# TheCacophonyProject/classifier-pipeline

Hardware: AMD Instinct MI355X
Metric: CPTV frames/s end-to-end (track+classify) at 160x120 (higher is better)
Workload: dtype u16/i32 track stage (f32 normalise, f64 gates); f32 crop/tile; f32 CNN (stride-1 3x3 convs of stages 2-4 (+ the stride-2 one): two fp16 planes per operand rounded to nearest (11 + 11 significand bits), power-of-two range scaling, 3 fp16 MFMAs per K step, device-side rerun in the exact split if an ac

## Files before the change

classifier-pipeline_amd/csrc/cpx_cnn_rw.hip:

```cpp
#include <hip/hip_runtime.h>

#include <algorithm>
#include <type_traits>

#include "cpx_conv_layout_core.h"
#include "cpx_kernels.h"

namespace cpx {

namespace {

typedef unsigned u32x4 __attribute__((ext_vector_type(4)));
typedef float f32x4 __attribute__((ext_vector_type(4)));
typedef _Float16 f16x2 __attribute__((ext_vector_type(2)));
typedef _Float16 f16x8 __attribute__((ext_vector_type(8)));

template <typename T>
__device__ __forceinline__ const T* at_off(const T* base, unsigned bytes) {
  return reinterpret_cast<const T*>(reinterpret_cast<const char*>(base) + bytes);
}
template <typename T>
__device__ __forceinline__ T* at_off(T* base, unsigned bytes) {
  return reinterpret_cast<T*>(reinterpret_cast<char*>(base) + bytes);
}
__device__ __forceinline__ unsigned pix_off(int y, int x, int W, int C) {
  return __umul24(__umul24((unsigned)y, (unsigned)W) + (unsigned)x, (unsigned)C);
}
__device__ __forceinline__ float relu_bits(float x) { return __int_as_float(max(__float_as_int(x), 0)); }
__device__ __forceinline__ void split_h(float a, float b, unsigned& hi, unsigned& lo) {
  f16x2 v = {(_Float16)a, (_Float16)b};
  hi = __builtin_bit_cast(unsigned, v);
  asm("v_fma_mixlo_f16 %0, %1, 1.0, -%2 op_sel:[0,0,0] op_sel_hi:[0,0,1]" : "=v"(lo) : "v"(a), "v"(hi));
  asm("v_fma_mixhi_f16 %0, %1, 1.0, -%2 op_sel:[0,0,1] op_sel_hi:[0,0,1]" : "+v"(lo) : "v"(b), "v"(hi));
}
__device__ __forceinline__ f32x4 mfma_h(u32x4 w, u32x4 x, f32x4 c) {
  return __builtin_amdgcn_mfma_f32_16x16x32_f16(__builtin_bit_cast(f16x8, w), __builtin_bit_cast(f16x8, x), c, 0, 0, 0);
}

struct RwTiles {
  unsigned long long m_tx, m_ty;
  int tiles_x, tiles_y, total;
};
template <int I, int N, typename F>
__device__ __forceinline__ void static_for(F&& f) {
  if constexpr (I < N) {
    f(std::integral_constant<int, I>{});
    static_for<I + 1, N>(f);
  }
}
__device__ __forceinline__ int div_magic(int n, unsigned long long m) { return (int)(((unsigned long long)n * m) >> 42); }

constexpr int RW_TW = 16;
constexpr int RW_CT = 256;
constexpr int RW_PPI = RW_CT / 8;
constexpr int RW_WC = 64;

template <int S, int NCH, int ROWS>
struct RwGeo {
  static constexpr int PW = 15 * S + 3, PH = (ROWS - 1) * S + 3, NPX = PH * PW;
  static constexpr int NP = (NPX * 8 + RW_CT - 1) / RW_CT;
  static constexpr int NPXP = (NP * RW_PPI + 3) / 4 * 4 + 2;
  static constexpr int BUF = 2 * 2 * NPXP * 2;
  static constexpr int STEPS = 3 * PH;
  static constexpr int CING = 32 * NCH;
  static constexpr size_t LDS = (size_t)2 * BUF * 16 + (size_t)(2 * CING + 3 * RW_WC) * sizeof(float);
};
constexpr int SC_NPXP = 258;
constexpr int SC_ITEMS = 16 * RW_TW * 8 / RW_CT;
constexpr size_t SC_LDS = (size_t)2 * 2 * SC_NPXP * 2 * 16;

template <int S, int NCH, int ROWS, bool BN, bool RES, bool SC = false>
__global__ __launch_bounds__(RW_CT) __attribute__((amdgpu_waves_per_eu(1, 1))) void conv_rw_kernel(ConvArgs a, const uint4* __restrict__ wimg, RwTiles td) {
  using G = RwGeo<S, NCH, ROWS>;
  constexpr int PW = G::PW, NPX = G::NPX, NP = G::NP, NPXP = G::NPXP, BUF = G::BUF, STEPS = G::STEPS, CING = G::CING, PH = G::PH;
  static_assert(!SC || (S == 1 && NCH == 2 && ROWS == 16 && !RES), "the fp16 shortcut is built into the stride-1 form's two-chunk stream");
  if (*a.ovf != 0) return;
  extern __shared__ __attribute__((aligned(16))) uint4 lds4[];
  uint4* s_buf = lds4;
  float* s_bn = reinterpret_cast<float*>(lds4 + 2 * BUF);
  float* s_par = s_bn + 2 * CING;
  uint4* s_sc = reinterpret_cast<uint4*>(s_par + 3 * RW_WC);
  const int tid = threadIdx.x, lane = tid & 63, wave = tid >> 6, i16 = lane & 15, q = lane >> 4;
  const int ct = wave;
  const int cout_g = a.Cout / a.groups, nhalf = cout_g / RW_WC;
  const int g = blockIdx.y / nhalf, half = blockIdx.y - g * nhalf;
  constexpr bool has_bn = BN;

  u32x4 Wr[NCH][9][2];
  {
    const u32x4* wg = reinterpret_cast<const u32x4*>(wimg) + (size_t)g * NCH * 3 * 24 * cout_g + (q * cout_g + half * RW_WC + ct * 16 + i16);
#pragma unroll
    for (int c = 0; c < NCH; ++c)
#pragma unroll
      for (int ky = 0; ky < 3; ++ky)
#pragma unroll
        for (int kx = 0; kx < 3; ++kx)
#pragma unroll
          for (int p = 0; p < 2; ++p) Wr[c][ky * 3 + kx][p] = wg[(size_t)((c * 3 + ky) * 24 + (p * 3 + kx) * 4) * cout_g];
  }
  u32x4 Wsc[2];
  if constexpr (SC) {
    const u32x4* ws = reinterpret_cast<const u32x4*>(a.sc_planes) + (size_t)g * 8 * cout_g + (q * cout_g + half * RW_WC + ct * 16 + i16);
    Wsc[0] = ws[0];
    Wsc[1] = ws[(size_t)4 * cout_g];
  }
  if (tid < CING) {
    const int ci = g * CING + tid;
    s_bn[tid] = has_bn ? a.in_scale[ci] * a.act_scale : a.act_scale;
    s_bn[CING + tid] = has_bn ? a.in_shift[ci] * a.act_scale : 0.0f;
  }
  if (tid < RW_WC) {
    const int ch = g * cout_g + half * RW_WC + tid;
    float os = a.w_unscale[ch] * a.act_unscale;
    if (a.out_scale) os *= a.out_scale[ch];
    float ob = a.out_shift ? a.out_shift[ch] : 0.0f;
    if (a.sc_in && a.sc_bias) ob += a.sc_bias[ch];
    s_par[tid] = os;
    s_par[RW_WC + tid] = ob;
    s_par[2 * RW_WC + tid] = a.w_scale[ch] * a.act_scale;
  }

  const int per_xcd = (td.total + 7) >> 3;
  auto tile_of = [&](int t) { return (t & 7) * per_xcd + (t >> 3); };
  auto decode = [&](int tile, int& n_, int& oy_, int& ox_) {
    int qd = div_magic(tile, td.m_tx);
    ox_ = (tile - qd * td.tiles_x) * RW_TW;
    tile = qd;
    qd = div_magic(tile, td.m_ty);
    oy_ = (tile - qd * td.tiles_y) * ROWS;
    n_ = qd;
  };
  int t = blockIdx.x;
  while (t < 8 * per_xcd && tile_of(t) >= td.total) t += gridDim.x;
  if (t >= 8 * per_xcd) return;
  auto advance = [&](int& n_, int& oy_, int& ox_) {
    t += gridDim.x;
    const bool more = t < 8 * per_xcd && tile_of(t) < td.total;
    if (more) decode(tile_of(t), n_, oy_, ox_);
    return more;
  };
  int n0, oy0, ox0, n1, oy1, ox1, n2, oy2, ox2;
  decode(tile_of(t), n0, oy0, ox0);

  u32x4 pre_p[NP];
  const int q8 = tid & 7;
  int ipos[NP];
#pragma unroll
  for (int i = 0; i < NP; ++i) {
    const int px = min((tid >> 3) + RW_PPI * i, NPX - 1);
    const int py = px / PW;
    ipos[i] = (py << 8) | (px - py * PW);
  }
  const unsigned st_base = (unsigned)((((q8 >> 2) * NPXP + (tid >> 3)) * 4 + (q8 & 3)) * 8);
  f32x4 psc[NCH], psh[NCH];
  const unsigned coff0 = (unsigned)(g * CING + 4 * q8);
  auto med3 = [](int x, int lo, int hi) __attribute__((always_inline)) {
    int r;
    asm("v_med3_i32 %0, %1, %2, %3" : "=v"(r) : "v"(x), "v"(lo), "s"(hi));
    return r;
  };
  const int Hm1 = a.H - 1, Wm1 = a.W - 1;
  auto issue_item = [&](const int i, const int c, const int n_, const int oy_, const int ox_) __attribute__((always_inline)) {
    const float* in_n = a.in + (size_t)n_ * a.H * a.W * a.Cin;
    const int iy = oy_ * S - a.pad_top + (ipos[i] >> 8), ix = ox_ * S - a.pad_left + (ipos[i] & 0xFF);
    const int cy = med3(iy, 0, Hm1), cx = med3(ix, 0, Wm1);
    pre_p[i] = *reinterpret_cast<const u32x4*>(at_off(in_n, (pix_off(cy, cx, a.W, a.Cin) + coff0 + (unsigned)(c * 32)) << 2));
  };
  unsigned hmax = 0u;
  auto pk_max_u16 = [](unsigned x, unsigned y) __attribute__((always_inline)) {
    unsigned r;
    asm("v_pk_max_u16 %0, %1, %2" : "=v"(r) : "v"(x), "v"(y));
    return r;
  };
  auto activate_item = [&](const int i, const int c, const int oy_, const int ox_) __attribute__((always_inline)) {
    float v[4];
#pragma unroll
    for (int j = 0; j < 4; ++j) v[j] = __fmaf_rn(__uint_as_float(pre_p[i][j]), psc[c][j], psh[c][j]);
    if (has_bn) {
#pragma unroll
      for (int j = 0; j < 4; ++j) v[j] = fmaxf(v[j], 0.0f);
    }
    const int iy = oy_ * S - a.pad_top + (ipos[i] >> 8), ix = ox_ * S - a.pad_left + (ipos[i] & 0xFF);
    const bool inside = (unsigned)iy < (unsigned)a.H && (unsigned)ix < (unsigned)a.W;
#pragma unroll
    for (int j = 0; j < 4; ++j) pre_p[i][j] = __float_as_uint(inside ? v[j] : 0.0f);
  };
  auto store_item = [&](const int i, const int bsel) __attribute__((always_inline)) {
    unsigned h0, h1, l0, l1;
    split_h(__uint_as_float(pre_p[i][0]), __uint_as_float(pre_p[i][1]), h0, l0);
    split_h(__uint_as_float(pre_p[i][2]), __uint_as_float(pre_p[i][3]), h1, l1);
    if (has_bn) hmax = pk_max_u16(pk_max_u16(hmax, h0), h1);
    else hmax = pk_max_u16(pk_max_u16(hmax, h0 & 0x7FFF7FFFu), h1 & 0x7FFF7FFFu);
    unsigned char* sp = reinterpret_cast<unsigned char*>(s_buf) + st_base;
    *reinterpret_cast<uint2*>(sp + (bsel * BUF * 16 + i * (RW_PPI * 32))) = make_uint2(h0, h1);
    *reinterpret_cast<uint2*>(sp + (bsel * BUF * 16 + 2 * NPXP * 32 + i * (RW_PPI * 32))) = make_uint2(l0, l1);
  };

  u32x4 pre_s[SC ? SC_ITEMS : 1];
  u32x4 xsh[2], xsl[2];
  const unsigned sc_st_base = (unsigned)((((q8 >> 2) * SC_NPXP + (tid >> 3)) * 4 + (q8 & 3)) * 8);
  const int sc_a_base = ((q >> 1) * SC_NPXP + i16) * 2 + (q & 1);
  auto issue_sc = [&](const int i, const int n_, const int oy_, const int ox_) __attribute__((always_inline)) {
    if constexpr (SC) {
      const float* sc_n = a.sc_in + (size_t)n_ * a.sc_H * a.sc_W * a.sc_cin;
      const int oy = min(oy_ + 2 * i + (tid >> 7), a.Ho - 1), ox = min(ox_ + ((tid >> 3) & 15), a.Wo - 1);
      pre_s[i] = *reinterpret_cast<const u32x4*>(
          at_off(sc_n, (pix_off(oy * a.sc_stride, ox * a.sc_stride, a.sc_W, a.sc_cin) + (unsigned)(g * 32 + 4 * q8)) << 2));
    }
  };
  auto store_sc = [&](const int i) __attribute__((always_inline)) {
    if constexpr (SC) {
      unsigned h0, h1, l0, l1;
      split_h(__uint_as_float(pre_s[i][0]) * a.sc_xscale, __uint_as_float(pre_s[i][1]) * a.sc_xscale, h0, l0);
      split_h(__uint_as_float(pre_s[i][2]) * a.sc_xscale, __uint_as_float(pre_s[i][3]) * a.sc_xscale, h1, l1);
      hmax = pk_max_u16(pk_max_u16(hmax, h0 & 0x7FFF7FFFu), h1 & 0x7FFF7FFFu);
      unsigned char* sp = reinterpret_cast<unsigned char*>(s_sc) + sc_st_base;
      *reinterpret_cast<uint2*>(sp + i * (RW_PPI * 32)) = make_uint2(h0, h1);
      *reinterpret_cast<uint2*>(sp + (2 * SC_NPXP * 32 + i * (RW_PPI * 32))) = make_uint2(l0, l1);
    }
  };

  f32x4 acc[ROWS];
  const int ch_l = g * cout_g + half * RW_WC + ct * 16 + 4 * q;
  auto init_acc = [&]() __attribute__((always_inline)) {
#pragma unroll
    for (int o = 0; o < ROWS; ++o) acc[o] = f32x4{0.0f, 0.0f, 0.0f, 0.0f};
  };
  f32x4 rres[RES ? ROWS : 1];
  auto issue_res = [&](const int o, const int n_, const int oy_, const int ox_) __attribute__((always_inline)) {
    if constexpr (RES) {
      const float* res_n = a.residual + (size_t)n_ * a.Ho * a.Wo * a.Cout;
      const int ox = min(ox_ + i16, a.Wo - 1), oy = min(oy_ + o, a.Ho - 1);
      rres[o] = *reinterpret_cast<const f32x4*>(at_off(res_n, (pix_off(oy, ox, a.Wo, a.Cout) + (unsigned)ch_l) << 2));
    }
  };

  const int a_base = ((q >> 1) * NPXP + S * i16) * 2 + (q & 1);
  constexpr int RW_AHEAD = 3, RW_RING = RW_AHEAD + 1;
  auto compute = [&](auto cc, auto bc, auto&& between) __attribute__((always_inline)) {
    constexpr int C = decltype(cc)::value, B = decltype(bc)::value;
    const uint4* sb = s_buf + B * BUF + a_base;
    u32x4 xh[RW_RING], xl[RW_RING];
    auto frag = [&](auto sc) __attribute__((always_inline)) {
      constexpr int s = decltype(sc)::value;
      constexpr int kx = s / PH, i = s - PH * kx, bf = s % RW_RING;
      xh[bf] = __builtin_bit_cast(u32x4, sb[(i * PW + kx) * 2]);
      xl[bf] = __builtin_bit_cast(u32x4, sb[4 * NPXP + (i * PW + kx) * 2]);
    };
    static_for<0, RW_AHEAD>(frag);
    static_for<0, STEPS>([&](auto sc) __attribute__((always_inline)) {
      constexpr int s = decltype(sc)::value;
      constexpr int kx = s / PH, i = s - PH * kx, bf = s % RW_RING;
      if constexpr (s + RW_AHEAD < STEPS) frag(std::integral_constant<int, s + RW_AHEAD>{});
      static_for<0, 3>([&](auto pc) __attribute__((always_inline)) {
        constexpr int pr = decltype(pc)::value;
        static_for<0, 3>([&](auto rc) __attribute__((always_inline)) {
          constexpr int r = decltype(rc)::value, d = i - r, o = d / S;
          if constexpr (d >= 0 && d % S == 0 && o < ROWS) {
            if constexpr (pr == 0) acc[o] = mfma_h(Wr[C][r * 3 + kx][1], xh[bf], acc[o]);
            if constexpr (pr == 1) acc[o] = mfma_h(Wr[C][r * 3 + kx][0], xl[bf], acc[o]);
            if constexpr (pr == 2) acc[o] = mfma_h(Wr[C][r * 3 + kx][0], xh[bf], acc[o]);
          }
        });
      });
      between(sc);
      __builtin_amdgcn_sched_barrier(0);
    });
  };
  auto unit = [&](auto cc, auto bc, auto ccc, auto cic, auto lastc, const int oyc, const int oxc, const int ni, const int oyi,
                  const int oxi) __attribute__((always_inline)) {
    constexpr int B = decltype(bc)::value, CC = decltype(ccc)::value, CI = decltype(cic)::value;
    constexpr bool LAST = decltype(lastc)::value;
    compute(cc, bc, [&](auto sc) __attribute__((always_inline)) {
      constexpr int s = decltype(sc)::value;
      constexpr int jlo = (s * 3 * NP + STEPS - 1) / STEPS, jhi = ((s + 1) * 3 * NP + STEPS - 1) / STEPS;
      static_for<jlo, (jhi < 3 * NP ? jhi : 3 * NP)>([&](auto jc) __attribute__((always_inline)) {
        constexpr int j = decltype(jc)::value, i = j / 3, k = j % 3;
        if constexpr (k == 0) activate_item(i, CC, oyc, oxc);
        if constexpr (k == 1) store_item(i, B ^ 1);
        if constexpr (k == 2) issue_item(i, CI, ni, oyi, oxi);
      });
      if constexpr (SC && !LAST) {
        constexpr int klo = (s * SC_ITEMS + STEPS - 1) / STEPS, khi = ((s + 1) * SC_ITEMS + STEPS - 1) / STEPS;
        static_for<klo, (khi < SC_ITEMS ? khi : SC_ITEMS)>([&](auto kc) __attribute__((always_inline)) { store_sc(decltype(kc)::value); });
      }
      if constexpr (SC && LAST) {
        if constexpr (s % 3 == 0 && s >= 3 && s / 3 - 1 < ROWS) {
          constexpr int o = s / 3 - 1;
          acc[o] = mfma_h(Wsc[1], xsh[o & 1], acc[o]);
          acc[o] = mfma_h(Wsc[0], xsl[o & 1], acc[o]);
          acc[o] = mfma_h(Wsc[0], xsh[o & 1], acc[o]);
        }
        if constexpr (s % 3 == 0 && s / 3 < ROWS) {
          constexpr int o = s / 3;
          xsh[o & 1] = __builtin_bit_cast(u32x4, s_sc[sc_a_base + o * 2 * RW_TW]);
          xsl[o & 1] = __builtin_bit_cast(u32x4, s_sc[sc_a_base + 4 * SC_NPXP + o * 2 * RW_TW]);
        }
        constexpr int klo = (s * SC_ITEMS + STEPS - 1) / STEPS, khi = ((s + 1) * SC_ITEMS + STEPS - 1) / STEPS;
        static_for<klo, (khi < SC_ITEMS ? khi : SC_ITEMS)>([&](auto kc) __attribute__((always_inline)) { issue_sc(decltype(kc)::value, ni, oyi, oxi); });
      }
      if constexpr (LAST && RES) {
        constexpr int olo = (s * ROWS + STEPS - 1) / STEPS, ohi = ((s + 1) * ROWS + STEPS - 1) / STEPS;
        static_for<olo, (ohi < ROWS ? ohi : ROWS)>([&](auto oc) __attribute__((always_inline)) { issue_res(decltype(oc)::value, n0, oy0, ox0); });
      }
    });
  };

  auto finish = [&](const int n_, const int oy_, const int ox_) __attribute__((always_inline)) {
    const int ox = min(ox_ + i16, a.Wo - 1);
    if (!SC && a.sc_in) {
      const int sc_cg = a.sc_cin / a.groups;
      const float* wsc = a.sc_w + ((size_t)g * sc_cg + q) * cout_g + half * RW_WC + ct * 16 + i16;
      const float ss = s_par[2 * RW_WC + ct * 16 + i16];
      const float* sc_n = a.sc_in + (size_t)n_ * a.sc_H * a.sc_W * a.sc_cin + g * sc_cg + q;
      for (int k4 = 0; k4 < sc_cg; k4 += 4) {
        const float ws = wsc[(size_t)k4 * cout_g] * ss;
#pragma unroll
        for (int o = 0; o < ROWS; ++o) {
          const int oy = min(oy_ + o, a.Ho - 1);
          const float xs = sc_n[((size_t)(oy * a.sc_stride) * a.sc_W + ox * a.sc_stride) * a.sc_cin + k4];
          acc[o] = __builtin_amdgcn_mfma_f32_16x16x4f32(ws, xs, acc[o], 0, 0, 0);
        }
      }
    }
    float* out_n = a.out + (size_t)n_ * a.Ho * a.Wo * a.Cout;
    const f32x4 os = *reinterpret_cast<const f32x4*>(s_par + ct * 16 + 4 * q);
    const f32x4 ob = *reinterpret_cast<const f32x4*>(s_par + RW_WC + ct * 16 + 4 * q);
    const bool xok = ox_ + i16 < a.Wo;
    const unsigned off0 = (pix_off(min(oy_, a.Ho - 1), ox, a.Wo, a.Cout) + (unsigned)ch_l) << 2;
    const unsigned row_bytes = (unsigned)(a.Wo * a.Cout) << 2;
    const bool whole = oy_ + ROWS <= a.Ho;
    auto row = [&](const int o, const bool ok, const unsigned off) __attribute__((always_inline)) {
      f32x4 v;
#pragma unroll
      for (int j = 0; j < 4; ++j) v[j] = __fmaf_rn(acc[o][j], os[j], ob[j]);
      if constexpr (RES) v += rres[o];
      if (a.relu) {
        asm volatile("");
        v.x = relu_bits(v.x); v.y = relu_bits(v.y); v.z = relu_bits(v.z); v.w = relu_bits(v.w);
      }
      if (ok) *reinterpret_cast<f32x4*>(at_off(out_n, off)) = v;
    };
    if (whole) {
#pragma unroll
      for (int o = 0; o < ROWS; ++o) row(o, xok, off0 + (unsigned)o * row_bytes);
    } else {
#pragma unroll
      for (int o = 0; o < ROWS; ++o) row(o, xok && oy_ + o < a.Ho, off0 + (unsigned)min(o, a.Ho - 1 - oy_) * row_bytes);
    }
  };

#pragma unroll
  for (int i = 0; i < NP; ++i) issue_item(i, 0, n0, oy0, ox0);
  __syncthreads();
#pragma unroll
  for (int c = 0; c < NCH; ++c) {
    psc[c] = *reinterpret_cast<const f32x4*>(s_bn + c * 32 + 4 * q8);
    psh[c] = *reinterpret_cast<const f32x4*>(s_bn + CING + c * 32 + 4 * q8);
  }
#pragma unroll
  for (int i = 0; i < NP; ++i) {
    activate_item(i, 0, oy0, ox0);
    store_item(i, 0);
  }
  using I0 = std::integral_constant<int, 0>;
  using I1 = std::integral_constant<int, 1>;
  using Yes = std::integral_constant<bool, true>;
  using No = std::integral_constant<bool, false>;
  if constexpr (NCH == 2) {
#pragma unroll
    for (int i = 0; i < NP; ++i) issue_item(i, 1, n0, oy0, ox0);
    if constexpr (SC) {
#pragma unroll
      for (int i = 0; i < SC_ITEMS; ++i) issue_sc(i, n0, oy0, ox0);
    }
    init_acc();
    for (;;) {
      n1 = n0; oy1 = oy0; ox1 = ox0;
      const bool more = advance(n1, oy1, ox1);
      __syncthreads();
      unit(I0{}, I0{}, I1{}, I0{}, No{}, oy0, ox0, n1, oy1, ox1);
      __syncthreads();
      unit(I1{}, I1{}, I0{}, I1{}, Yes{}, oy1, ox1, n1, oy1, ox1);
      finish(n0, oy0, ox0);
      if (!more) break;
      n0 = n1; oy0 = oy1; ox0 = ox1;
      init_acc();
    }
  } else {
    n1 = n0; oy1 = oy0; ox1 = ox0;
    bool more1 = advance(n1, oy1, ox1);
#pragma unroll
    for (int i = 0; i < NP; ++i) issue_item(i, 0, n1, oy1, ox1);
    init_acc();
    for (;;) {
      n2 = n1; oy2 = oy1; ox2 = ox1;
      bool more2 = more1 && advance(n2, oy2, ox2);
      __syncthreads();
      unit(I0{}, I0{}, I0{}, I0{}, Yes{}, oy1, ox1, n2, oy2, ox2);
      finish(n0, oy0, ox0);
      if (!more1) break;
      n0 = n1; oy0 = oy1; ox0 = ox1; n1 = n2; oy1 = oy2; ox1 = ox2; more1 = more2;
      init_acc();
      n2 = n1; oy2 = oy1; ox2 = ox1;
      more2 = more1 && advance(n2, oy2, ox2);
      __syncthreads();
      unit(I0{}, I1{}, I0{}, I0{}, Yes{}, oy1, ox1, n2, oy2, ox2);
      finish(n0, oy0, ox0);
      if (!more1) break;
      n0 = n1; oy0 = oy1; ox0 = ox1; n1 = n2; oy1 = oy2; ox1 = ox2; more1 = more2;
      init_acc();
    }
  }
  if ((hmax & 0x7FFFu) >= 0x7C00u || ((hmax >> 16) & 0x7FFFu) >= 0x7C00u) atomicOr(a.ovf, 1);
}

__global__ __launch_bounds__(256) void split_shortcut_kernel(const float* __restrict__ w, uint4* __restrict__ out, int groups, int cin_g,
                                                             int cout_g, const float* __restrict__ wscale, float factor) {
  const int nch = cin_g / 32;
  const int total = groups * nch * 4 * cout_g;
  const int idx = blockIdx.x * blockDim.x + threadIdx.x;
  if (idx >= total) return;
  const int col = idx % cout_g;
  int r = idx / cout_g;
  const int qq = r & 3;
  r >>= 2;
  const int chunk = r % nch, g = r / nch;
  const float f = wscale[g * cout_g + col] * factor;
  float v[8];
#pragma unroll
  for (int j = 0; j < 8; ++j) v[j] = w[((size_t)g * cin_g + chunk * 32 + 8 * qq + j) * cout_g + col] * f;
  uint4 hi, lo;
  split_h(v[0], v[1], hi.x, lo.x);
  split_h(v[2], v[3], hi.y, lo.y);
  split_h(v[4], v[5], hi.z, lo.z);
  split_h(v[6], v[7], hi.w, lo.w);
  const size_t base = (size_t)(g * nch + chunk) * 8 * cout_g + (size_t)qq * cout_g + col;
  out[base] = hi;
  out[base + (size_t)4 * cout_g] = lo;
}

}

bool conv_shortcut_planes_layer(const ConvArgs& second, int sc_cin_g) {
  if (conv_rw_kind(second) == 1) return sc_cin_g == 32;
  return second.ksize == 3 && second.stride == 1 && second.groups >= 1 && second.Cin == second.Cout &&
         second.Cout == 128 * second.groups && sc_cin_g == 64;
}
size_t conv_shortcut_image_bytes(int groups, int cin_g, int cout_g) { return (size_t)groups * (cin_g / 32) * 8 * cout_g * 16; }
void launch_split_shortcut(const float* sc_w, void* img, int groups, int cin_g, int cout_g, const float* w_scale, float factor,
                           hipStream_t s) {
  const int total = groups * (cin_g / 32) * 4 * cout_g;
  hipLaunchKernelGGL(split_shortcut_kernel, dim3((unsigned)((total + 255) / 256)), dim3(256), 0, s, sc_w, reinterpret_cast<uint4*>(img),
                     groups, cin_g, cout_g, w_scale, factor);
}

int conv_rw_kind(const ConvArgs& a) { return conv_rw_kind_of(conv_shape_of(a)); }
bool conv_rw_layer(const ConvArgs& a) { return conv_rw_kind(a) == 1; }

namespace {
template <int S, int NCH, int ROWS, bool BN, bool RES, bool SC = false>
int launch_rw_t(const ConvArgs& a, const uint4* wimg, hipStream_t s) {
  using G = RwGeo<S, NCH, ROWS>;
  constexpr size_t LDS = G::LDS + (SC ? SC_LDS : 0);
  static_assert(LDS <= 160 * 1024 - 1024, "two chunk buffers (and the shortcut's operand) must fit the CU's LDS");
  RwTiles td{};
  if (const int rc = fill_tiles(td, (a.Wo + RW_TW - 1) / RW_TW, (a.Ho + ROWS - 1) / ROWS, a.N, TILES_PERSISTENT)) return rc;
  static bool lds_ready[64];
  if (!cpx_dyn_lds_ready(reinterpret_cast<const void*>(conv_rw_kernel<S, NCH, ROWS, BN, RES, SC>), lds_ready, 160 * 1024 - 1024)) return -1;
  const int cus = cpx_device_cus();
  if (cus == 0) return -1;
  const int ny = a.groups * ((a.Cout / a.groups) / RW_WC);
  const int gx = persistent_grid_x(cus, ny, td.total);
  hipLaunchKernelGGL((conv_rw_kernel<S, NCH, ROWS, BN, RES, SC>), dim3((unsigned)gx, (unsigned)ny), dim3(RW_CT), LDS, s, a, wimg, td);
  return 0;
}
}

int launch_conv_rw(const ConvArgs& a, const void* wimg, hipStream_t s) {
  const int kind = conv_rw_kind(a);
  if (!kind || !a.half || a.planes != 2 || a.ovf == nullptr || a.in_planes || a.out_planes) return -2;
  if ((long long)a.H * a.W >= (1 << 24) || (long long)a.Ho * a.Wo >= (1 << 24)) return -3;
  if (a.sc_in && ((a.sc_cin / a.groups) & 3)) return -2;
  const uint4* wi = reinterpret_cast<const uint4*>(wimg);
  const bool bn = a.in_scale != nullptr, res = a.residual != nullptr;
  if (kind == 1) {
    if (a.pad_top != 1 || a.pad_left != 1 || a.H != a.Ho || a.W != a.Wo) return -2;
    if (a.sc_in && a.sc_planes) {
      if (bn || res || !conv_shortcut_planes_layer(a, a.sc_cin / a.groups) || a.sc_stride < 1 || !(a.sc_xscale > 0.0f) ||
          (a.sc_H - 1) / a.sc_stride + 1 != a.Ho || (a.sc_W - 1) / a.sc_stride + 1 != a.Wo)
        return -2;
      if ((long long)a.sc_H * a.sc_W >= (1 << 24) || (long long)a.sc_H * a.sc_W * a.sc_cin >= (1ll << 30)) return -3;
      return launch_rw_t<1, 2, 16, false, false, true>(a, wi, s);
    }
    if (bn && res) return launch_rw_t<1, 2, 16, true, true>(a, wi, s);
    if (bn) return launch_rw_t<1, 2, 16, true, false>(a, wi, s);
    if (res) return launch_rw_t<1, 2, 16, false, true>(a, wi, s);
    return launch_rw_t<1, 2, 16, false, false>(a, wi, s);
  }
  if (res || a.sc_in || a.pad_top < 0 || a.pad_top > 1 || a.pad_left < 0 || a.pad_left > 1) return -2;
  if (kind == 2) return bn ? launch_rw_t<2, 1, 8, true, false>(a, wi, s) : launch_rw_t<2, 1, 8, false, false>(a, wi, s);
  return bn ? launch_rw_t<3, 2, 4, true, false>(a, wi, s) : launch_rw_t<3, 2, 4, false, false>(a, wi, s);
}

}
```

classifier-pipeline_amd/csrc/cpx_conv_layout_core.h:

```cpp
#pragma once
#include <stddef.h>

#include <algorithm>

namespace cpx {

struct ConvShape { int groups, cin_g, cout_g, ksize, stride; };
template <class Args>
ConvShape conv_shape_of(const Args& a) {
  if (a.groups < 1 || a.Cin % a.groups || a.Cout % a.groups) return ConvShape{};
  return ConvShape{a.groups, a.Cin / a.groups, a.Cout / a.groups, a.ksize, a.stride};
}

enum class ConvClass { Unsupported, Plain, Flat, Wide, C8, Stride2Rw, Rw3 };

inline ConvClass conv_class(const ConvShape& s) {
  if (s.ksize != 3) return ConvClass::Unsupported;
  if (s.stride == 3 && s.cin_g == 64 && s.cout_g == 128) return ConvClass::Rw3;
  if (s.stride == 2 && s.cin_g == 32 && s.cout_g == 64) return ConvClass::Stride2Rw;
  if (s.stride == 1 && s.cin_g == 8 && s.cout_g == 32) return ConvClass::C8;
  const bool c32_64 = s.cout_g == 32 || s.cout_g == 64;
  if (s.stride == 1 && (s.cin_g == 32 || s.cin_g == 64) && c32_64) return ConvClass::Wide;
  if (s.cin_g < 16 || s.cin_g % 16) return ConvClass::Unsupported;
  if ((s.stride == 1 && s.cout_g == 128) || (s.stride == 2 && s.cout_g == 64)) return ConvClass::Flat;
  return s.stride == 1 && c32_64 ? ConvClass::Plain : ConvClass::Unsupported;
}
inline int conv_rw_kind_of(const ConvShape& s) {
  switch (conv_class(s)) {
    case ConvClass::Wide: return s.cin_g == 64 && s.cout_g == 64 ? 1 : 0;
    case ConvClass::Stride2Rw: return 2;
    case ConvClass::Rw3: return 3;
    default: return 0;
  }
}

struct WeightImages {
  static constexpr size_t absent = ~(size_t)0;
  static constexpr size_t C8_HALF_ENTRIES = 3 * 2 * 4 * 32;
  ConvClass cls = ConvClass::Unsupported;
  int chunk = 0;
  size_t planes3 = absent, planes2 = absent, half = absent, scales = absent, rw_half = absent, bytes = 0;

  static WeightImages of(const ConvShape& s) {
    WeightImages l;
    l.cls = conv_class(s);
    if (l.cls == ConvClass::Unsupported) return l;
    const auto put = [&l](size_t& image, size_t size) { image = l.bytes; l.bytes += size; };
    const size_t row = (size_t)s.cout_g * 16;
    const size_t scales = ((size_t)2 * s.groups * s.cout_g * sizeof(float) + 15) / 16 * 16;
    if (l.cls == ConvClass::C8) {
      put(l.planes3, (size_t)s.groups * 30 * row);
      put(l.half, (size_t)s.groups * C8_HALF_ENTRIES * 16);
      put(l.scales, scales);
      return l;
    }
    l.chunk = l.cls == ConvClass::Wide || l.cls == ConvClass::Rw3 ? 32 : 16;
    const auto image = [&](int planes) { return (size_t)s.groups * (s.cin_g / l.chunk) * (9 * l.chunk / 8 * planes) * row; };
    if (l.cls != ConvClass::Rw3) put(l.planes3, image(3));
    if (l.cls == ConvClass::Plain) return l;
    if (l.cls != ConvClass::Rw3) put(l.planes2, image(2));
    put(l.half, image(2));
    put(l.scales, scales);
    if (l.cls == ConvClass::Stride2Rw) put(l.rw_half, image(2));
    return l;
  }
};

constexpr int TILE_AXIS_LIMIT = 4096;
constexpr long long TILES_PER_LAUNCH = 1ll << 22;
constexpr long long TILES_PERSISTENT = (1ll << 22) - 8;
inline unsigned long long tile_magic(int d) { return (1ull << 42) / (unsigned long long)d + 1; }

template <class Tiles>
int fill_tiles(Tiles& td, int tiles_x, int tiles_y, long long n, long long limit) {
  if (tiles_x < 1 || tiles_y < 1 || tiles_x >= TILE_AXIS_LIMIT || tiles_y >= TILE_AXIS_LIMIT) return -3;
  const long long total = (long long)tiles_x * tiles_y * n;
  if (total >= limit) return -3;
  td.tiles_x = tiles_x, td.m_tx = tile_magic(tiles_x);
  td.tiles_y = tiles_y, td.m_ty = tile_magic(tiles_y);
  td.total = (int)total;
  return 0;
}
template <class Tiles>
int fill_tiles(Tiles& td, int tiles_x, int tiles_y, long long n, int nsplit, long long limit) {
  if (nsplit < 1 || nsplit >= TILE_AXIS_LIMIT) return -3;
  td.nsplit = nsplit, td.m_nsplit = tile_magic(nsplit);
  return fill_tiles(td, tiles_x, tiles_y, n * nsplit, limit);
}

inline int persistent_grid_x(int cus, int ny, long long tiles) {
  const int gx = std::max(8, cus / std::max(ny, 1) / 8 * 8);
  return (int)std::min<long long>(gx, (tiles + 7) / 8 * 8);
}

#if defined(__HIPCC__)
#define CPX_WALK_HD __host__ __device__ __forceinline__
#else
#define CPX_WALK_HD inline
#endif
enum { WALK_TILES = 0, WALK_ROWS = 1 };
struct BlkTiles {
  unsigned long long m_tx, m_ty;
  int tiles_x, tiles_y, total;
  int walk, units;
};
CPX_WALK_HD int tile_div(int n, unsigned long long m) { return (int)(((unsigned long long)n * m) >> 42); }
inline void set_walk(BlkTiles& td, int walk) {
  td.walk = walk;
  td.units = walk == WALK_ROWS ? td.total / td.tiles_x : td.total;
}
CPX_WALK_HD bool walk_tile(const BlkTiles& td, int bx, int gx, int j, int& n, int& ty, int& tx) {
  int col = 0;
  if (td.walk == WALK_ROWS) {
    const int jr = tile_div(j, td.m_tx);
    col = j - jr * td.tiles_x;
    j = jr;
  }
  const int per_xcd = (td.units + 7) >> 3;
  const int t = bx + j * gx;
  if (t >= 8 * per_xcd) return false;
  int unit = (t & 7) * per_xcd + (t >> 3);
  if (unit >= td.units) return false;
  if (td.walk == WALK_ROWS) {
    tx = td.tiles_x - 1 - col;
  } else {
    const int qd = tile_div(unit, td.m_tx);
    tx = unit - qd * td.tiles_x;
    unit = qd;
  }
  n = tile_div(unit, td.m_ty);
  ty = unit - n * td.tiles_y;
  return true;
}
inline long long walk_max_tiles(const BlkTiles& td, int walk, int gx) {
  const long long units = walk == WALK_ROWS ? td.total / td.tiles_x : td.total;
  const long long per_xcd = (units + 7) / 8, wgs = gx / 8;
  return (per_xcd + wgs - 1) / wgs * (walk == WALK_ROWS ? td.tiles_x : 1);
}
constexpr double WALK_CARRY_SAVING = 0.06;
inline int choose_walk(const BlkTiles& td, int gx) {
  const double rows = (double)walk_max_tiles(td, WALK_ROWS, gx) / td.tiles_x * (td.tiles_x - WALK_CARRY_SAVING * (td.tiles_x - 1));
  return rows < (double)walk_max_tiles(td, WALK_TILES, gx) ? WALK_ROWS : WALK_TILES;
}

}
```

Measured before the change: 3.114 million.

## Compute two output-channel tiles per wave in the stride-3 rw conv

Result: no change. 3.144 million (median of 6 runs) (+1.0%).

```diff
diff --git a/classifier-pipeline_amd/csrc/cpx_cnn_rw.hip b/classifier-pipeline_amd/csrc/cpx_cnn_rw.hip
--- a/classifier-pipeline_amd/csrc/cpx_cnn_rw.hip
+++ b/classifier-pipeline_amd/csrc/cpx_cnn_rw.hip
@@ -1,6 +1,7 @@
 #include <hip/hip_runtime.h>
 
 #include <algorithm>
+#include <cstdlib>
 #include <type_traits>
 
 #include "cpx_conv_layout_core.h"
@@ -35,6 +36,16 @@
 }
 __device__ __forceinline__ f32x4 mfma_h(u32x4 w, u32x4 x, f32x4 c) {
   return __builtin_amdgcn_mfma_f32_16x16x32_f16(__builtin_bit_cast(f16x8, w), __builtin_bit_cast(f16x8, x), c, 0, 0, 0);
+}
+
+template <int B>
+__device__ __forceinline__ int add_byte(int base, int packed) {
+  int r;
+  if constexpr (B == 0) asm("v_add_u32_sdwa %0, %1, %2 dst_sel:DWORD dst_unused:UNUSED_PAD src0_sel:DWORD src1_sel:BYTE_0" : "=v"(r) : "s"(base), "v"(packed));
+  if constexpr (B == 1) asm("v_add_u32_sdwa %0, %1, %2 dst_sel:DWORD dst_unused:UNUSED_PAD src0_sel:DWORD src1_sel:BYTE_1" : "=v"(r) : "s"(base), "v"(packed));
+  if constexpr (B == 2) asm("v_add_u32_sdwa %0, %1, %2 dst_sel:DWORD dst_unused:UNUSED_PAD src0_sel:DWORD src1_sel:BYTE_2" : "=v"(r) : "s"(base), "v"(packed));
+  if constexpr (B == 3) asm("v_add_u32_sdwa %0, %1, %2 dst_sel:DWORD dst_unused:UNUSED_PAD src0_sel:DWORD src1_sel:BYTE_3" : "=v"(r) : "s"(base), "v"(packed));
+  return r;
 }
 
 struct RwTiles {
@@ -55,7 +66,7 @@
 constexpr int RW_PPI = RW_CT / 8;
 constexpr int RW_WC = 64;
 
-template <int S, int NCH, int ROWS>
+template <int S, int NCH, int ROWS, int NCT = 1>
 struct RwGeo {
   static constexpr int PW = 15 * S + 3, PH = (ROWS - 1) * S + 3, NPX = PH * PW;
   static constexpr int NP = (NPX * 8 + RW_CT - 1) / RW_CT;
@@ -63,15 +74,17 @@
   static constexpr int BUF = 2 * 2 * NPXP * 2;
   static constexpr int STEPS = 3 * PH;
   static constexpr int CING = 32 * NCH;
-  static constexpr size_t LDS = (size_t)2 * BUF * 16 + (size_t)(2 * CING + 3 * RW_WC) * sizeof(float);
+  static constexpr size_t LDS = (size_t)2 * BUF * 16 + (size_t)(2 * CING + 3 * RW_WC * NCT) * sizeof(float);
 };
 constexpr int SC_NPXP = 258;
 constexpr int SC_ITEMS = 16 * RW_TW * 8 / RW_CT;
 constexpr size_t SC_LDS = (size_t)2 * 2 * SC_NPXP * 2 * 16;
 
-template <int S, int NCH, int ROWS, bool BN, bool RES, bool SC = false>
+template <int S, int NCH, int ROWS, bool BN, bool RES, bool SC = false, int NCT = 1>
 __global__ __launch_bounds__(RW_CT) __attribute__((amdgpu_waves_per_eu(1, 1))) void conv_rw_kernel(ConvArgs a, const uint4* __restrict__ wimg, RwTiles td) {
-  using G = RwGeo<S, NCH, ROWS>;
+  using G = RwGeo<S, NCH, ROWS, NCT>;
+  constexpr int WC = RW_WC * NCT;
+  static_assert(NCT == 1 || (NCT == 2 && !RES && !SC), "two column tiles per wave: the forms without a residual or a fused shortcut");
   constexpr int PW = G::PW, NPX = G::NPX, NP = G::NP, NPXP = G::NPXP, BUF = G::BUF, STEPS = G::STEPS, CING = G::CING, PH = G::PH;
   static_assert(!SC || (S == 1 && NCH == 2 && ROWS == 16 && !RES), "the fp16 shortcut is built into the stride-1 form's two-chunk stream");
   if (*a.ovf != 0) return;
@@ -79,16 +92,17 @@
   uint4* s_buf = lds4;
   float* s_bn = reinterpret_cast<float*>(lds4 + 2 * BUF);
   float* s_par = s_bn + 2 * CING;
-  uint4* s_sc = reinterpret_cast<uint4*>(s_par + 3 * RW_WC);
+  uint4* s_sc = reinterpret_cast<uint4*>(s_par + 3 * WC);
   const int tid = threadIdx.x, lane = tid & 63, wave = tid >> 6, i16 = lane & 15, q = lane >> 4;
   const int ct = wave;
-  const int cout_g = a.Cout / a.groups, nhalf = cout_g / RW_WC;
+  const int cout_g = a.Cout / a.groups, nhalf = cout_g / WC;
   const int g = blockIdx.y / nhalf, half = blockIdx.y - g * nhalf;
   constexpr bool has_bn = BN;
 
-  u32x4 Wr[NCH][9][2];
-  {
-    const u32x4* wg = reinterpret_cast<const u32x4*>(wimg) + (size_t)g * NCH * 3 * 24 * cout_g + (q * cout_g + half * RW_WC + ct * 16 + i16);
+  u32x4 Wr[NCT][NCH][9][2];
+#pragma unroll
+  for (int j = 0; j < NCT; ++j) {
+    const u32x4* wg = reinterpret_cast<const u32x4*>(wimg) + (size_t)g * NCH * 3 * 24 * cout_g + (q * cout_g + half * WC + j * RW_WC + ct * 16 + i16);
 #pragma unroll
     for (int c = 0; c < NCH; ++c)
 #pragma unroll
@@ -96,11 +110,11 @@
 #pragma unroll
         for (int kx = 0; kx < 3; ++kx)
 #pragma unroll
-          for (int p = 0; p < 2; ++p) Wr[c][ky * 3 + kx][p] = wg[(size_t)((c * 3 + ky) * 24 + (p * 3 + kx) * 4) * cout_g];
+          for (int p = 0; p < 2; ++p) Wr[j][c][ky * 3 + kx][p] = wg[(size_t)((c * 3 + ky) * 24 + (p * 3 + kx) * 4) * cout_g];
   }
   u32x4 Wsc[2];
   if constexpr (SC) {
-    const u32x4* ws = reinterpret_cast<const u32x4*>(a.sc_planes) + (size_t)g * 8 * cout_g + (q * cout_g + half * RW_WC + ct * 16 + i16);
+    const u32x4* ws = reinterpret_cast<const u32x4*>(a.sc_planes) + (size_t)g * 8 * cout_g + (q * cout_g + half * WC + ct * 16 + i16);
     Wsc[0] = ws[0];
     Wsc[1] = ws[(size_t)4 * cout_g];
   }
@@ -109,15 +123,15 @@
     s_bn[tid] = has_bn ? a.in_scale[ci] * a.act_scale : a.act_scale;
     s_bn[CING + tid] = has_bn ? a.in_shift[ci] * a.act_scale : 0.0f;
   }
-  if (tid < RW_WC) {
-    const int ch = g * cout_g + half * RW_WC + tid;
+  if (tid < WC) {
+    const int ch = g * cout_g + half * WC + tid;
     float os = a.w_unscale[ch] * a.act_unscale;
     if (a.out_scale) os *= a.out_scale[ch];
     float ob = a.out_shift ? a.out_shift[ch] : 0.0f;
     if (a.sc_in && a.sc_bias) ob += a.sc_bias[ch];
     s_par[tid] = os;
-    s_par[RW_WC + tid] = ob;
-    s_par[2 * RW_WC + tid] = a.w_scale[ch] * a.act_scale;
+    s_par[WC + tid] = ob;
+    s_par[2 * WC + tid] = a.w_scale[ch] * a.act_scale;
   }
 
   const int per_xcd = (td.total + 7) >> 3;
@@ -144,15 +158,31 @@
 
   u32x4 pre_p[NP];
   const int q8 = tid & 7;
-  int ipos[NP];
+  constexpr int IPK = NCT == 1 ? 1 : 2;
+  int ipos[(NP + IPK - 1) / IPK];
 #pragma unroll
   for (int i = 0; i < NP; ++i) {
     const int px = min((tid >> 3) + RW_PPI * i, NPX - 1);
     const int py = px / PW;
-    ipos[i] = (py << 8) | (px - py * PW);
-  }
+    const int v = (py << 8) | (px - py * PW);
+    if (IPK == 1 || (i & 1) == 0) ipos[i / IPK] = v;
+    else ipos[i / IPK] |= v << 16;
+  }
+  auto pos_y = [&](const int i, const int base) __attribute__((always_inline)) {
+    if constexpr (IPK == 1) return base + (ipos[i] >> 8);
+    else return i % IPK ? add_byte<3>(base, ipos[i / IPK]) : add_byte<1>(base, ipos[i / IPK]);
+  };
+  auto pos_x = [&](const int i, const int base) __attribute__((always_inline)) {
+    if constexpr (IPK == 1) return base + (ipos[i] & 0xFF);
+    else return i % IPK ? add_byte<2>(base, ipos[i / IPK]) : add_byte<0>(base, ipos[i / IPK]);
+  };
   const unsigned st_base = (unsigned)((((q8 >> 2) * NPXP + (tid >> 3)) * 4 + (q8 & 3)) * 8);
-  f32x4 psc[NCH], psh[NCH];
+  constexpr bool PSC_UNIT = NCT == 2;
+  f32x4 psc[PSC_UNIT ? 1 : NCH], psh[PSC_UNIT ? 1 : NCH];
+  auto load_bn = [&](const int slot, const int c) __attribute__((always_inline)) {
+    psc[slot] = *reinterpret_cast<const f32x4*>(s_bn + c * 32 + 4 * q8);
+    psh[slot] = *reinterpret_cast<const f32x4*>(s_bn + CING + c * 32 + 4 * q8);
+  };
   const unsigned coff0 = (unsigned)(g * CING + 4 * q8);
   auto med3 = [](int x, int lo, int hi) __attribute__((always_inline)) {
     int r;
@@ -162,7 +192,7 @@
   const int Hm1 = a.H - 1, Wm1 = a.W - 1;
   auto issue_item = [&](const int i, const int c, const int n_, const int oy_, const int ox_) __attribute__((always_inline)) {
     const float* in_n = a.in + (size_t)n_ * a.H * a.W * a.Cin;
-    const int iy = oy_ * S - a.pad_top + (ipos[i] >> 8), ix = ox_ * S - a.pad_left + (ipos[i] & 0xFF);
+    const int iy = pos_y(i, oy_ * S - a.pad_top), ix = pos_x(i, ox_ * S - a.pad_left);
     const int cy = med3(iy, 0, Hm1), cx = med3(ix, 0, Wm1);
     pre_p[i] = *reinterpret_cast<const u32x4*>(at_off(in_n, (pix_off(cy, cx, a.W, a.Cin) + coff0 + (unsigned)(c * 32)) << 2));
   };
@@ -175,12 +205,12 @@
   auto activate_item = [&](const int i, const int c, const int oy_, const int ox_) __attribute__((always_inline)) {
     float v[4];
 #pragma unroll
-    for (int j = 0; j < 4; ++j) v[j] = __fmaf_rn(__uint_as_float(pre_p[i][j]), psc[c][j], psh[c][j]);
+    for (int j = 0; j < 4; ++j) v[j] = __fmaf_rn(__uint_as_float(pre_p[i][j]), psc[PSC_UNIT ? 0 : c][j], psh[PSC_UNIT ? 0 : c][j]);
     if (has_bn) {
 #pragma unroll
       for (int j = 0; j < 4; ++j) v[j] = fmaxf(v[j], 0.0f);
     }
-    const int iy = oy_ * S - a.pad_top + (ipos[i] >> 8), ix = ox_ * S - a.pad_left + (ipos[i] & 0xFF);
+    const int iy = pos_y(i, oy_ * S - a.pad_top), ix = pos_x(i, ox_ * S - a.pad_left);
     const bool inside = (unsigned)iy < (unsigned)a.H && (unsigned)ix < (unsigned)a.W;
 #pragma unroll
     for (int j = 0; j < 4; ++j) pre_p[i][j] = __float_as_uint(inside ? v[j] : 0.0f);
@@ -220,11 +250,13 @@
     }
   };
 
-  f32x4 acc[ROWS];
-  const int ch_l = g * cout_g + half * RW_WC + ct * 16 + 4 * q;
+  f32x4 acc[NCT][ROWS];
+  const int ch_l = g * cout_g + half * WC + ct * 16 + 4 * q;
   auto init_acc = [&]() __attribute__((always_inline)) {
 #pragma unroll
-    for (int o = 0; o < ROWS; ++o) acc[o] = f32x4{0.0f, 0.0f, 0.0f, 0.0f};
+    for (int j = 0; j < NCT; ++j)
+#pragma unroll
+      for (int o = 0; o < ROWS; ++o) acc[j][o] = f32x4{0.0f, 0.0f, 0.0f, 0.0f};
   };
   f32x4 rres[RES ? ROWS : 1];
   auto issue_res = [&](const int o, const int n_, const int oy_, const int ox_) __attribute__((always_inline)) {
@@ -236,7 +268,7 @@
   };
 
   const int a_base = ((q >> 1) * NPXP + S * i16) * 2 + (q & 1);
-  constexpr int RW_AHEAD = 3, RW_RING = RW_AHEAD + 1;
+  constexpr int RW_AHEAD = NCT == 1 ? 3 : 2, RW_RING = RW_AHEAD + 1;
   auto compute = [&](auto cc, auto bc, auto&& between) __attribute__((always_inline)) {
     constexpr int C = decltype(cc)::value, B = decltype(bc)::value;
     const uint4* sb = s_buf + B * BUF + a_base;
@@ -257,9 +289,12 @@
         static_for<0, 3>([&](auto rc) __attribute__((always_inline)) {
           constexpr int r = decltype(rc)::value, d = i - r, o = d / S;
           if constexpr (d >= 0 && d % S == 0 && o < ROWS) {
-            if constexpr (pr == 0) acc[o] = mfma_h(Wr[C][r * 3 + kx][1], xh[bf], acc[o]);
-            if constexpr (pr == 1) acc[o] = mfma_h(Wr[C][r * 3 + kx][0], xl[bf], acc[o]);
-            if constexpr (pr == 2) acc[o] = mfma_h(Wr[C][r * 3 + kx][0], xh[bf], acc[o]);
+            static_for<0, NCT>([&](auto jc) __attribute__((always_inline)) {
+              constexpr int j = decltype(jc)::value;
+              if constexpr (pr == 0) acc[j][o] = mfma_h(Wr[j][C][r * 3 + kx][1], xh[bf], acc[j][o]);
+              if constexpr (pr == 1) acc[j][o] = mfma_h(Wr[j][C][r * 3 + kx][0], xl[bf], acc[j][o]);
+              if constexpr (pr == 2) acc[j][o] = mfma_h(Wr[j][C][r * 3 + kx][0], xh[bf], acc[j][o]);
+            });
           }
         });
       });
@@ -267,10 +302,14 @@
       __builtin_amdgcn_sched_barrier(0);
     });
   };
+  constexpr int DEFER = NCT == 2 ? 6 : 0;
+  static_assert(DEFER == 0 || NCH == 2, "the deferred requests name the other chunk");
+  int dn = 0, doy = 0, dox = 0;
   auto unit = [&](auto cc, auto bc, auto ccc, auto cic, auto lastc, const int oyc, const int oxc, const int ni, const int oyi,
                   const int oxi) __attribute__((always_inline)) {
     constexpr int B = decltype(bc)::value, CC = decltype(ccc)::value, CI = decltype(cic)::value;
     constexpr bool LAST = decltype(lastc)::value;
+    if constexpr (PSC_UNIT) load_bn(0, CC);
     compute(cc, bc, [&](auto sc) __attribute__((always_inline)) {
       constexpr int s = decltype(sc)::value;
       constexpr int jlo = (s * 3 * NP + STEPS - 1) / STEPS, jhi = ((s + 1) * 3 * NP + STEPS - 1) / STEPS;
@@ -278,7 +317,10 @@
         constexpr int j = decltype(jc)::value, i = j / 3, k = j % 3;
         if constexpr (k == 0) activate_item(i, CC, oyc, oxc);
         if constexpr (k == 1) store_item(i, B ^ 1);
-        if constexpr (k == 2) issue_item(i, CI, ni, oyi, oxi);
+        if constexpr (k == 2) {
+          if constexpr (i >= DEFER) issue_item(i - DEFER, CI, ni, oyi, oxi);
+          else issue_item(i - DEFER + NP, CI ^ 1, dn, doy, dox);
+        }
       });
       if constexpr (SC && !LAST) {
         constexpr int klo = (s * SC_ITEMS + STEPS - 1) / STEPS, khi = ((s + 1) * SC_ITEMS + STEPS - 1) / STEPS;
@@ -287,9 +329,9 @@
       if constexpr (SC && LAST) {
         if constexpr (s % 3 == 0 && s >= 3 && s / 3 - 1 < ROWS) {
           constexpr int o = s / 3 - 1;
-          acc[o] = mfma_h(Wsc[1], xsh[o & 1], acc[o]);
-          acc[o] = mfma_h(Wsc[0], xsl[o & 1], acc[o]);
-          acc[o] = mfma_h(Wsc[0], xsh[o & 1], acc[o]);
+          acc[0][o] = mfma_h(Wsc[1], xsh[o & 1], acc[0][o]);
+          acc[0][o] = mfma_h(Wsc[0], xsl[o & 1], acc[0][o]);
+          acc[0][o] = mfma_h(Wsc[0], xsh[o & 1], acc[0][o]);
         }
         if constexpr (s % 3 == 0 && s / 3 < ROWS) {
           constexpr int o = s / 3;
@@ -310,53 +352,61 @@
     const int ox = min(ox_ + i16, a.Wo - 1);
     if (!SC && a.sc_in) {
       const int sc_cg = a.sc_cin / a.groups;
-      const float* wsc = a.sc_w + ((size_t)g * sc_cg + q) * cout_g + half * RW_WC + ct * 16 + i16;
-      const float ss = s_par[2 * RW_WC + ct * 16 + i16];
       const float* sc_n = a.sc_in + (size_t)n_ * a.sc_H * a.sc_W * a.sc_cin + g * sc_cg + q;
-      for (int k4 = 0; k4 < sc_cg; k4 += 4) {
-        const float ws = wsc[(size_t)k4 * cout_g] * ss;
-#pragma unroll
-        for (int o = 0; o < ROWS; ++o) {
-          const int oy = min(oy_ + o, a.Ho - 1);
-          const float xs = sc_n[((size_t)(oy * a.sc_stride) * a.sc_W + ox * a.sc_stride) * a.sc_cin + k4];
-          acc[o] = __builtin_amdgcn_mfma_f32_16x16x4f32(ws, xs, acc[o], 0, 0, 0);
+#pragma unroll
+      for (int j = 0; j < NCT; ++j) {
+        const float* wsc = a.sc_w + ((size_t)g * sc_cg + q) * cout_g + half * WC + j * RW_WC + ct * 16 + i16;
+        const float ss = s_par[2 * WC + j * RW_WC + ct * 16 + i16];
+        for (int k4 = 0; k4 < sc_cg; k4 += 4) {
+          const float ws = wsc[(size_t)k4 * cout_g] * ss;
+#pragma unroll
+          for (int o = 0; o < ROWS; ++o) {
+            const int oy = min(oy_ + o, a.Ho - 1);
+            const float xs = sc_n[((size_t)(oy * a.sc_stride) * a.sc_W + ox * a.sc_stride) * a.sc_cin + k4];
+            acc[j][o] = __builtin_amdgcn_mfma_f32_16x16x4f32(ws, xs, acc[j][o], 0, 0, 0);
+          }
         }
       }
     }
     float* out_n = a.out + (size_t)n_ * a.Ho * a.Wo * a.Cout;
-    const f32x4 os = *reinterpret_cast<const f32x4*>(s_par + ct * 16 + 4 * q);
-    const f32x4 ob = *reinterpret_cast<const f32x4*>(s_par + RW_WC + ct * 16 + 4 * q);
     const bool xok = ox_ + i16 < a.Wo;
     const unsigned off0 = (pix_off(min(oy_, a.Ho - 1), ox, a.Wo, a.Cout) + (unsigned)ch_l) << 2;
     const unsigned row_bytes = (unsigned)(a.Wo * a.Cout) << 2;
     const bool whole = oy_ + ROWS <= a.Ho;
-    auto row = [&](const int o, const bool ok, const unsigned off) __attribute__((always_inline)) {
-      f32x4 v;
-#pragma unroll
-      for (int j = 0; j < 4; ++j) v[j] = __fmaf_rn(acc[o][j], os[j], ob[j]);
-      if constexpr (RES) v += rres[o];
-      if (a.relu) {
-        asm volatile("");
-        v.x = relu_bits(v.x); v.y = relu_bits(v.y); v.z = relu_bits(v.z); v.w = relu_bits(v.w);
+#pragma unroll
+    for (int j = 0; j < NCT; ++j) {
+      const f32x4 os = *reinterpret_cast<const f32x4*>(s_par + j * RW_WC + ct * 16 + 4 * q);
+      const f32x4 ob = *reinterpret_cast<const f32x4*>(s_par + WC + j * RW_WC + ct * 16 + 4 * q);
+      auto row = [&](const int o, const bool ok, const unsigned off) __attribute__((always_inline)) {
+        f32x4 v;
+#pragma unroll
+        for (int k = 0; k < 4; ++k) v[k] = __fmaf_rn(acc[j][o][k], os[k], ob[k]);
+        if constexpr (RES) v += rres[o];
+        if (a.relu) {
+          asm volatile("");
+          v.x = relu_bits(v.x); v.y = relu_bits(v.y); v.z = relu_bits(v.z); v.w = relu_bits(v.w);
+        }
+        if (ok) *reinterpret_cast<f32x4*>(at_off(out_n, off)) = v;
+      };
+      const unsigned offj = off0 + (unsigned)(j * RW_WC * 4);
+      if (whole) {
+#pragma unroll
+        for (int o = 0; o < ROWS; ++o) row(o, xok, offj + (unsigned)o * row_bytes);
+      } else {
+#pragma unroll
+        for (int o = 0; o < ROWS; ++o) row(o, xok && oy_ + o < a.Ho, offj + (unsigned)min(o, a.Ho - 1 - oy_) * row_bytes);
       }
-      if (ok) *reinterpret_cast<f32x4*>(at_off(out_n, off)) = v;
-    };
-    if (whole) {
-#pragma unroll
-      for (int o = 0; o < ROWS; ++o) row(o, xok, off0 + (unsigned)o * row_bytes);
-    } else {
-#pragma unroll
-      for (int o = 0; o < ROWS; ++o) row(o, xok && oy_ + o < a.Ho, off0 + (unsigned)min(o, a.Ho - 1 - oy_) * row_bytes);
     }
   };
 
 #pragma unroll
   for (int i = 0; i < NP; ++i) issue_item(i, 0, n0, oy0, ox0);
   __syncthreads();
-#pragma unroll
-  for (int c = 0; c < NCH; ++c) {
-    psc[c] = *reinterpret_cast<const f32x4*>(s_bn + c * 32 + 4 * q8);
-    psh[c] = *reinterpret_cast<const f32x4*>(s_bn + CING + c * 32 + 4 * q8);
+  if constexpr (PSC_UNIT) {
+    load_bn(0, 0);
+  } else {
+#pragma unroll
+    for (int c = 0; c < NCH; ++c) load_bn(c, c);
   }
 #pragma unroll
   for (int i = 0; i < NP; ++i) {
@@ -379,8 +429,10 @@
       n1 = n0; oy1 = oy0; ox1 = ox0;
       const bool more = advance(n1, oy1, ox1);
       __syncthreads();
+      if constexpr (DEFER != 0) { dn = n0; doy = oy0; dox = ox0; }
       unit(I0{}, I0{}, I1{}, I0{}, No{}, oy0, ox0, n1, oy1, ox1);
       __syncthreads();
+      if constexpr (DEFER != 0) { dn = n1; doy = oy1; dox = ox1; }
       unit(I1{}, I1{}, I0{}, I1{}, Yes{}, oy1, ox1, n1, oy1, ox1);
       finish(n0, oy0, ox0);
       if (!more) break;
@@ -459,20 +511,21 @@
 bool conv_rw_layer(const ConvArgs& a) { return conv_rw_kind(a) == 1; }
 
 namespace {
-template <int S, int NCH, int ROWS, bool BN, bool RES, bool SC = false>
+template <int S, int NCH, int ROWS, bool BN, bool RES, bool SC = false, int NCT = 1>
 int launch_rw_t(const ConvArgs& a, const uint4* wimg, hipStream_t s) {
-  using G = RwGeo<S, NCH, ROWS>;
+  using G = RwGeo<S, NCH, ROWS, NCT>;
+  static_assert(RW_WC * NCT == conv_rw_wg_channels(NCT) && RW_CT == 64 * CONV_RW_WAVES, "cpx_conv_layout_core.h states the workgroup");
   constexpr size_t LDS = G::LDS + (SC ? SC_LDS : 0);
   static_assert(LDS <= 160 * 1024 - 1024, "two chunk buffers (and the shortcut's operand) must fit the CU's LDS");
   RwTiles td{};
   if (const int rc = fill_tiles(td, (a.Wo + RW_TW - 1) / RW_TW, (a.Ho + ROWS - 1) / ROWS, a.N, TILES_PERSISTENT)) return rc;
   static bool lds_ready[64];
-  if (!cpx_dyn_lds_ready(reinterpret_cast<const void*>(conv_rw_kernel<S, NCH, ROWS, BN, RES, SC>), lds_ready, 160 * 1024 - 1024)) return -1;
+  if (!cpx_dyn_lds_ready(reinterpret_cast<const void*>(conv_rw_kernel<S, NCH, ROWS, BN, RES, SC, NCT>), lds_ready, 160 * 1024 - 1024)) return -1;
   const int cus = cpx_device_cus();
   if (cus == 0) return -1;
-  const int ny = a.groups * ((a.Cout / a.groups) / RW_WC);
+  const int ny = conv_rw_grid_y(conv_shape_of(a), NCT);
   const int gx = persistent_grid_x(cus, ny, td.total);
-  hipLaunchKernelGGL((conv_rw_kernel<S, NCH, ROWS, BN, RES, SC>), dim3((unsigned)gx, (unsigned)ny), dim3(RW_CT), LDS, s, a, wimg, td);
+  hipLaunchKernelGGL((conv_rw_kernel<S, NCH, ROWS, BN, RES, SC, NCT>), dim3((unsigned)gx, (unsigned)ny), dim3(RW_CT), LDS, s, a, wimg, td);
   return 0;
 }
 }
@@ -500,6 +553,9 @@
   }
   if (res || a.sc_in || a.pad_top < 0 || a.pad_top > 1 || a.pad_left < 0 || a.pad_left > 1) return -2;
   if (kind == 2) return bn ? launch_rw_t<2, 1, 8, true, false>(a, wi, s) : launch_rw_t<2, 1, 8, false, false>(a, wi, s);
+  const char* ew = std::getenv("CPX_RW_STRIDE3_WIDE");
+  if (conv_rw_column_tiles(kind, !ew || std::atoi(ew) != 0) == 2)
+    return bn ? launch_rw_t<3, 2, 4, true, false, false, 2>(a, wi, s) : launch_rw_t<3, 2, 4, false, false, false, 2>(a, wi, s);
   return bn ? launch_rw_t<3, 2, 4, true, false>(a, wi, s) : launch_rw_t<3, 2, 4, false, false>(a, wi, s);
 }
 
diff --git a/classifier-pipeline_amd/csrc/cpx_conv_layout_core.h b/classifier-pipeline_amd/csrc/cpx_conv_layout_core.h
--- a/classifier-pipeline_amd/csrc/cpx_conv_layout_core.h
+++ b/classifier-pipeline_amd/csrc/cpx_conv_layout_core.h
@@ -33,6 +33,11 @@
     default: return 0;
   }
 }
+
+constexpr int CONV_RW_WAVES = 4;
+constexpr int conv_rw_wg_channels(int nct) { return 16 * CONV_RW_WAVES * nct; }
+inline int conv_rw_column_tiles(int kind, bool wide) { return kind == 3 && wide ? 2 : 1; }
+inline int conv_rw_grid_y(const ConvShape& s, int nct) { return s.groups * (s.cout_g / conv_rw_wg_channels(nct)); }
 
 struct WeightImages {
   static constexpr size_t absent = ~(size_t)0;
```
